# carlosmwh1985/BspAtom

Hardware: AMD Instinct MI355X
Metric: l-channel eigensolves/sec at N_bsp=4096 fp64 (higher is better)
Workload: dtype f64; 1 GPU; Hydrogen Coulomb l=0..127, N_bsp=4096, k=9, KIND_GRID=0 rb=800 (BASELINE configs[3]); `value` = weak scaling: 128 l-channels per GPU, 128 in total; channels_total=128, eigenvector_owner_rank=0, collective_calls=0, launched_by=python

## Files before the change

bspatom_amd/csrc/common.h:

```cpp
#pragma once
#include <hip/hip_runtime.h>
#include <cstdint>
#include <cstdio>
#include <cstdlib>

#define BSP_OK 0
#define BSP_ERR_HIP (-1)
#define BSP_ERR_ARG (-2)
#define BSP_ERR_BSPLVB (-3)
#define BSP_ERR_NOGPU (-4)
#define BSP_ERR_UNSUPPORTED (-5)

#define BSP_HIP(x)                                                                          \
    do {                                                                                    \
        hipError_t e_ = (x);                                                                \
        if (e_ != hipSuccess) {                                                             \
            fprintf(stderr, "bspatom: HIP error '%s' at %s:%d\n", hipGetErrorString(e_),    \
                    __FILE__, __LINE__);                                                    \
            return BSP_ERR_HIP;                                                             \
        }                                                                                   \
    } while (0)

typedef double double4_t __attribute__((ext_vector_type(4)));

__host__ __device__ inline size_t ab_stride(int npad) { return (size_t)npad * 128 + 1088; }

namespace bsp {

struct Options {
    int sb2st_version = 0;
    int sb2st_ring = 0;
    int sb2st_margin = 3, sb2st_hyst = 2;
    int sb2st_lead = 0;
    int sb2st_check = 0;
    int sb2st_diag = 0;
    int sb2st_force_abort = 0;
    int sy2sb_groups = 2, sy2sb_lookahead = 1, sy2sb_segs = 0;
    int panel_qr = 3;
    int tsqr_max_m = 2048;
    int tsqr_regcap = 1;
    int gemm_diag = 0;
    int bisect = 3, bisect_ept = 0;
    int bisect_secant = 1;
    int bisect_tail = 1;
    int no_eigvec_prefetch = 0;
    int vec_early = 1;
    int vec_own_cu = 1;
    int sb2sb_mfma = 1;
    int sb16_rows = 1;
    int poison_c = 0;
    int route = 0;
    int fused_probe = 0;
    int cw_items4 = 1;
    int cw_nw = 1;
    int cw_streams = 2;
    int cw_chunk_min = 1024;
    int s_overlap = 1;
    int cw_diag = 0;
    int cw_split = 0;
    int cw_band8 = 1;
    int sb8_wgs = 0;
    int cw_ipw = 0;
    int cw_ldspad = 0;
    int cw_onediv = 0;
    int ktime = 0;
};
Options &opts();

int process_device();
int process_device_check(int device);
void process_device_latch(int device);

enum KSlot { KS_SYR2K = 0, KS_SYMM, KS_PANEL_QR, KS_CHAIN, KS_SB2SB, KS_SB16ST, KS_BISECT, KS_STDFORM, KS_CRAWFORD, KS_COUNT };
void ktime_begin(int slot, hipStream_t st);
void ktime_end(int slot, hipStream_t st);
struct KScope {
    int slot; hipStream_t st; bool on;
    KScope(int slot_, hipStream_t st_) : slot(slot_), st(st_), on(opts().ktime != 0) { if (on) ktime_begin(slot, st); }
    ~KScope() { if (on) ktime_end(slot, st); }
};

struct GemmDesc {
    int M, N, K, batch;
    const double *A; long sAm, sAk, bA;
    const double *B; long sBk, sBn, bB;
    double *C; long sCm, sCn, bC;
    double alpha, beta;
    int lower_only;
    int yoff;
    int ksplit;
    int kchunk;
    long bCs;
    int nsb, toff;
    int sbpre[80];
    int sbxy[80];
};
int gemm_f64(const GemmDesc &g, hipStream_t st);
int gemm_splitk_f64(const GemmDesc &g, int splits, double *part, hipStream_t st);
int tsmm64_f64(int m, int batch, const double *A, long lda, long bsA, const double *B, long bsB, double *C, long ldc, long bsC,
               double alpha, double beta, hipStream_t st);
int syr2k_lower_f64(int m, int batch, double *A22, long ld, long bsA, const double *buf, long ldb, long bsBuf, int seg, int nseg,
                    int part, hipStream_t st);
int symm_lower_f64(int m, int batch, const double *A22, long ld, long bsA, const double *W, long ldw, long bsW,
                   double *Y, long ldy, long bsY, hipStream_t st);

int launch_point_table(int nkp, int k, int ka, int nfun, const double *d_rt, const double *d_aind,
                       const double *d_xg, const double *d_wg, const double *d_vpot, double *d_ptab,
                       int *d_left, int *d_status, hipStream_t st);
int launch_assemble_bands(int nfun, int k, int ka, int nkp, int kind_pot, const double *d_bl, int l0,
                          int nl, const double *d_ptab, const int *d_left, double *d_SB, double *d_HB,
                          hipStream_t st);
int launch_dipole_bands(int nfun, int k, int ka, int nkp, const double *d_ptab, const int *d_left, double *d_RB,
                        hipStream_t st);
int launch_band_cholesky(int n, int k, const double *d_SB, double *d_UB, double *d_rdiag, int *d_info,
                         hipStream_t st);
int launch_band_cholesky_range(int n, int k, int jstart, int jstop, const double *d_SB, double *d_UB, double *d_rdiag, int *d_info,
                               hipStream_t st);
int launch_band_cholesky_pair(int n, int k, int jstop, const double *d_SB, double *d_UB, double *d_rdiag, int *d_info, hipStream_t st);
int launch_standard_form(int n, int npad, int k, int nl, const double *d_HB, const double *d_UB,
                         const double *d_rdiag, double *d_Y, double *d_C, hipStream_t st, int full = 0);
struct CrawfordWork {
    double *SBf, *UBf, *rdiagf;
    double *Qel, *LiB;
    double *D, *E, *G;
    int *info;
};
bool crawford_supported(int n, int k);
size_t crawford_work_bytes(int n, int k, int nl);
void crawford_carve(void *base, int n, int k, int nl, CrawfordWork *w);
constexpr int CW_CHUNKS = 4;
int crawford_prepare(int n, int k, const double *d_SB, const CrawfordWork &w, hipStream_t st, hipEvent_t *evc = nullptr);
int crawford_run(int n, int npad, int k, int nl, const double *d_SB, const double *d_HB, const CrawfordWork &w, double *d_AB,
                 hipStream_t st, bool s_prepared = false, hipEvent_t *evc = nullptr, hipStream_t aux0 = nullptr);
long tsqr_scr_doubles(int npad);
long tsqr_cntr_ints(int npad);
int tsqr_panel(int npad, int r0, int c0, int batch, double *d_A, double *buf, double *W, double *scr, int *cntr, hipStream_t st);
struct Sy2sbWork {
    double *tsqr_scr;
    int *tsqr_cntr;
    double *buf2;
    double *tau2;
    double *buf;
    double *W;
    double *G;
    double *T;
    double *Kmat;
    double *tau;
    double *part;
};
constexpr int SY2SB_SPLITK = 16;
size_t sy2sb_work_bytes(int npad, int nb, int batch);
void sy2sb_carve(void *base, int npad, int nb, int batch, Sy2sbWork *w);
int sy2sb_run(int npad, int nb, int batch, double *d_A, const Sy2sbWork &w, hipStream_t st);
int sy2sb_panel_only(int npad, int c0, int batch, double *d_A, const Sy2sbWork &w, hipStream_t st);
int launch_extract_band(int npad, int nb, int batch, const double *d_A, double *d_AB, hipStream_t st);
size_t sb2st_ctl_bytes(int batch);
int launch_sb2sb(int n, int npad, int batch, double *d_AB, hipStream_t st);
int launch_sb16st(int n, int npad, int batch, double *d_AB, double *d_d, double *d_e, hipStream_t st, int *d_status = nullptr,
                  void *ctl = nullptr, int hb = 16);
int launch_sb2st(int n, int npad, int b, int batch, double *d_AB, double *d_d, double *d_e,
                 hipStream_t st, int *d_status = nullptr, void *ctl = nullptr);
int launch_bisect(int n, int ldn, int batch, const double *d_d, const double *d_e, double *d_w,
                  long ldw, hipStream_t st);
int launch_bisect_one(int n, const double *d_d, const double *d_e, int m, double *d_out, hipStream_t st);
int launch_band_multisect(int n, int k, const double *d_SB, const double *d_HB, int m, double *d_out, hipStream_t st);
constexpr size_t OWN_CU_LDS = 144 * 1024;
int launch_early_vector(int n, int k, const double *d_SB, const double *d_HB, int m, double *d_E, double *d_work, double *d_vec,
                        int *d_info, hipStream_t st, bool own_cu);
int launch_inverse_iteration(int n, int k, int nvec, const double *d_SB, const double *d_HB,
                             const int *d_chan, const double *d_E, double *d_work, double *d_vec,
                             int *d_info, hipStream_t st);
size_t invit_work_doubles(int n, int k);
size_t invit_batch_slot_doubles(int n, int k);
int invit_batch_slots(int k, int items, int *slots);
int launch_inverse_iteration_batch(int n, int k, int count, int items, int slots, const double *d_SB, const double *d_HB,
                                   const double *d_E, double *d_work, double *d_vec, int *d_info, hipStream_t st);
int launch_band_apply(int n, int k, const double *d_RB, const double a[3], const double *d_x, double *d_v, hipStream_t st);
int launch_dots(int n, int m, const double *d_Z, const double *d_v, double *d_D, hipStream_t st);
int launch_wf_tabulate(int nkp, int k, int n, const double *d_rt, const double *d_c, double ra,
                       double rb, int npts, double *d_r, double *d_u, int *d_status, hipStream_t st);

struct PipeBufs {
    double *UB, *rdiag, *Y, *C, *AB, *d, *e;
    void *work;
    int *info;
    int *status = nullptr;
    void *sbctl = nullptr;
    void *cwork = nullptr;
    hipEvent_t *s_events = nullptr;
    hipStream_t aux0 = nullptr;
    hipEvent_t chase_after = nullptr;
};
int pipeline_route(int n, int k);
size_t pipe_bytes_per_channel(int npad);
int pipeline_enqueue(int n, int npad, int k, int nl, const double *d_SB, const double *d_HB,
                     const PipeBufs &b, double *d_Eout, hipStream_t st, hipEvent_t *ev, bool with_bisect = true, bool s_prepared = false);

}
```

bspatom_amd/csrc/tridiag.hip:

```cpp
#include <vector>
#include "common.h"

namespace bsp {

__device__ __forceinline__ int sturm_count(const double *__restrict__ d, const double *__restrict__ e2,
                                           int n, double x, double pivmin)
{
    double q = d[0] - x;
    if (fabs(q) < pivmin) q = -pivmin;
    int cnt = (q < 0.0) ? 1 : 0;
    for (int i = 1; i < n; ++i) {
        q = (d[i] - x) - e2[i - 1] / q;
        if (fabs(q) < pivmin) q = -pivmin;
        cnt += (q < 0.0) ? 1 : 0;
    }
    return cnt;
}

constexpr int EPT = 4;

__global__ __launch_bounds__(256) void bisect_kernel(int n, int ldn, const double *__restrict__ dall,
                                                    const double *__restrict__ eall, double *wall, long ldw)
{
    extern __shared__ double sm[];
    double *d = sm, *e2 = sm + n;
    __shared__ double red[8];
    const int tid = threadIdx.x;
    const size_t ch = blockIdx.y;
    const double *dg = dall + ch * (size_t)ldn, *eg = eall + ch * (size_t)ldn;
    double gl = 1e300, gu = -1e300, emax = 0.0;
    for (int i = tid; i < n; i += 256) {
        const double di = dg[i];
        const double el = (i > 0) ? fabs(eg[i - 1]) : 0.0;
        const double er = (i < n - 1) ? fabs(eg[i]) : 0.0;
        d[i] = di;
        e2[i] = (i < n - 1) ? eg[i] * eg[i] : 0.0;
        gl = fmin(gl, di - el - er);
        gu = fmax(gu, di + el + er);
        emax = fmax(emax, er * er);
    }
#pragma unroll
    for (int off = 32; off >= 1; off >>= 1) {
        gl = fmin(gl, __shfl_xor(gl, off));
        gu = fmax(gu, __shfl_xor(gu, off));
        emax = fmax(emax, __shfl_xor(emax, off));
    }
    if ((tid & 63) == 0) { red[tid >> 6] = gl; red[4 + (tid >> 6)] = gu; }
    __syncthreads();
    gl = fmin(fmin(red[0], red[1]), fmin(red[2], red[3]));
    gu = fmax(fmax(red[4], red[5]), fmax(red[6], red[7]));
    __syncthreads();
    if ((tid & 63) == 0) red[tid >> 6] = emax;
    __syncthreads();
    emax = fmax(fmax(red[0], red[1]), fmax(red[2], red[3]));
    const double safmin = 2.2250738585072014e-308;
    const double pivmin = safmin * fmax(1.0, emax);
    const double tnorm = fmax(fabs(gl), fabs(gu));
    const double eps = 2.220446049250313e-16;
    gl = gl - 2.1 * tnorm * eps * n - 2.1 * pivmin;
    gu = gu + 2.1 * tnorm * eps * n + 2.1 * pivmin;

    const int mbase = blockIdx.x * (256 * EPT) + tid;
    double lo[EPT], hi[EPT];
#pragma unroll
    for (int c = 0; c < EPT; ++c) { lo[c] = gl; hi[c] = gu; }
    for (int it = 0; it < 128; ++it) {
        double mid[EPT];
        bool done[EPT];
        bool alld = true;
#pragma unroll
        for (int c = 0; c < EPT; ++c) {
            mid[c] = 0.5 * (lo[c] + hi[c]);
            done[c] = (mid[c] <= lo[c]) || (mid[c] >= hi[c]) ||
                      (hi[c] - lo[c] <= 2.0 * eps * fmax(fabs(lo[c]), fabs(hi[c])) + 2.0 * pivmin);
            alld = alld && done[c];
        }
        if (__syncthreads_and(alld)) break;
        double q[EPT];
        int cnt[EPT];
        {
            const double d0 = d[0];
#pragma unroll
            for (int c = 0; c < EPT; ++c) {
                q[c] = d0 - mid[c];
                if (fabs(q[c]) < pivmin) q[c] = -pivmin;
                cnt[c] = (q[c] < 0.0) ? 1 : 0;
            }
        }
        for (int i = 1; i < n; ++i) {
            const double di = d[i], ei = e2[i - 1];
#pragma unroll
            for (int c = 0; c < EPT; ++c) {
                double r = __builtin_amdgcn_rcp(q[c]);
                r = r * (2.0 - q[c] * r);
                q[c] = (di - mid[c]) - ei * r;
                if (fabs(q[c]) < pivmin) q[c] = -pivmin;
                cnt[c] += (q[c] < 0.0) ? 1 : 0;
            }
        }
#pragma unroll
        for (int c = 0; c < EPT; ++c) {
            if (!done[c]) {
                if (cnt[c] > mbase + 256 * c) hi[c] = mid[c]; else lo[c] = mid[c];
            }
        }
    }
#pragma unroll
    for (int c = 0; c < EPT; ++c) {
        const int m = mbase + 256 * c;
        if (m < n) wall[ch * (size_t)ldw + m] = 0.5 * (lo[c] + hi[c]);
    }
}

constexpr int RS = 8;

__global__ __launch_bounds__(256) void bisect2_kernel(int n, int ldn, const double *__restrict__ dall,
                                                     const double *__restrict__ eall, double *wall, long ldw)
{
    extern __shared__ double sm[];
    const int np = (n + RS - 1) / RS * RS;
    double *d = sm, *e2 = sm + np + RS;
    __shared__ double red[8];
    const int tid = threadIdx.x;
    const size_t ch = blockIdx.y;
    const double *dg = dall + ch * (size_t)ldn, *eg = eall + ch * (size_t)ldn;
    double gl = 1e300, gu = -1e300;
    for (int i = tid; i < n; i += 256) {
        const double di = dg[i];
        const double el = (i > 0) ? fabs(eg[i - 1]) : 0.0;
        const double er = (i < n - 1) ? fabs(eg[i]) : 0.0;
        gl = fmin(gl, di - el - er);
        gu = fmax(gu, di + el + er);
    }
#pragma unroll
    for (int off = 32; off >= 1; off >>= 1) {
        gl = fmin(gl, __shfl_xor(gl, off));
        gu = fmax(gu, __shfl_xor(gu, off));
    }
    if ((tid & 63) == 0) { red[tid >> 6] = gl; red[4 + (tid >> 6)] = gu; }
    __syncthreads();
    gl = fmin(fmin(red[0], red[1]), fmin(red[2], red[3]));
    gu = fmax(fmax(red[4], red[5]), fmax(red[6], red[7]));
    const double eps = 2.220446049250313e-16;
    double tnorm = fmax(fabs(gl), fabs(gu));
    if (!(tnorm > 0.0)) tnorm = 1.0;
    int kexp;
    (void)frexp(tnorm, &kexp);
    const double sc = ldexp(1.0, -kexp), isc = ldexp(1.0, kexp);
    for (int i = tid; i < np + RS; i += 256) {
        d[i] = (i < n) ? dg[i] * sc : 2.0;
        const double ev = (i < n - 1) ? (eg[i] * sc) : 0.0;
        e2[i] = fmax(ev * ev, 1e-60);
    }
    __syncthreads();
    gl = gl * sc - 2.1 * eps * n - 1e-300;
    gu = gu * sc + 2.1 * eps * n + 1e-300;

    const int mbase = blockIdx.x * (256 * EPT) + tid;
    double lo[EPT], hi[EPT];
#pragma unroll
    for (int c = 0; c < EPT; ++c) { lo[c] = gl; hi[c] = gu; }
    for (int it = 0; it < 128; ++it) {
        double mid[EPT];
        bool done[EPT];
        bool alld = true;
#pragma unroll
        for (int c = 0; c < EPT; ++c) {
            mid[c] = 0.5 * (lo[c] + hi[c]);
            done[c] = (mid[c] <= lo[c]) || (mid[c] >= hi[c]) ||
                      (hi[c] - lo[c] <= 2.0 * eps * fmax(fabs(lo[c]), fabs(hi[c])) + 1e-300);
            alld = alld && done[c];
        }
        if (__syncthreads_and(alld)) break;
        double p0[EPT], p1[EPT];
        int cnt[EPT];
#pragma unroll
        for (int c = 0; c < EPT; ++c) { p0[c] = 1.0; p1[c] = d[0] - mid[c]; cnt[c] = (p1[c] < 0.0) ? 1 : 0; }
        for (int ib = 0; ib < np; ib += RS) {
#pragma unroll
            for (int r = 0; r < RS; ++r) {
                const int i = ib + r + 1;
                const double di = d[i], ei = e2[i - 1];
#pragma unroll
                for (int c = 0; c < EPT; ++c) {
                    const double pn = __builtin_fma(di - mid[c], p1[c], -(ei * p0[c]));
                    cnt[c] += (int)((unsigned)(__double2hiint(pn) ^ __double2hiint(p1[c])) >> 31);
                    p0[c] = p1[c];
                    p1[c] = pn;
                }
            }
#pragma unroll
            for (int c = 0; c < EPT; ++c) {
                int ea, eb;
                (void)frexp(p1[c], &ea);
                (void)frexp(p0[c], &eb);
                const int ex = (p1[c] == 0.0) ? eb : ((p0[c] == 0.0) ? ea : max(ea, eb));
                p1[c] = ldexp(p1[c], -ex);
                p0[c] = ldexp(p0[c], -ex);
            }
        }
#pragma unroll
        for (int c = 0; c < EPT; ++c) {
            if (!done[c]) {
                if (cnt[c] > mbase + 256 * c) hi[c] = mid[c]; else lo[c] = mid[c];
            }
        }
    }
#pragma unroll
    for (int c = 0; c < EPT; ++c) {
        const int m = mbase + 256 * c;
        if (m < n) wall[ch * (size_t)ldw + m] = 0.5 * (lo[c] + hi[c]) * isc;
    }
}

constexpr int HW = 32;

#define STURM_BLOCK(LOADROW)                                                                          \
    {                                                                                                 \
        _Pragma("unroll") for (int sb = 0; sb < HW / RS; ++sb) {                                      \
            _Pragma("unroll") for (int r = 0; r < RS; ++r) {                                          \
                const double2 v = LOADROW(ib + sb * RS + r + 1);                                      \
                _Pragma("unroll") for (int c = 0; c < EPT; ++c) {                                     \
                    const double pn = __builtin_fma(v.x - x[c], p1[c], -(v.y * p0[c]));               \
                    h[c] = __builtin_amdgcn_alignbit(h[c], (unsigned)__double2hiint(pn), 31);         \
                    p0[c] = p1[c];                                                                    \
                    p1[c] = pn;                                                                       \
                }                                                                                     \
            }                                                                                         \
            _Pragma("unroll") for (int c = 0; c < EPT; ++c) {                                         \
                const int ex = -__builtin_amdgcn_frexp_exp(p1[c]);      \
                p1[c] = __builtin_amdgcn_ldexp(p1[c], ex);                                            \
                p0[c] = __builtin_amdgcn_ldexp(p0[c], ex);                                            \
                if (VAL) es[c] -= ex;                                            \
            }                                                                                         \
        }                                                                                             \
        _Pragma("unroll") for (int c = 0; c < EPT; ++c) {                                             \
            const unsigned t = __builtin_amdgcn_alignbit(hp[c], h[c], 1);                             \
            cnt[c] += __builtin_popcount(h[c] ^ t);                                                   \
            hp[c] = h[c];                                                                             \
        }                                                                                             \
    }
__device__ __forceinline__ double2 sturm_gload(const double2 *p)
{
    typedef double d2v __attribute__((ext_vector_type(2)));
    const d2v v = __builtin_nontemporal_load(reinterpret_cast<const d2v *>(p));
    return make_double2(v.x, v.y);
}
template <int EPT, bool VAL = false>
__device__ __forceinline__ void sturm_counts3(const double2 *__restrict__ de, int np, const double (&x)[EPT], int (&cnt)[EPT],
                                              const double2 *__restrict__ gt = nullptr, int nl = 0x7fffffff, float *lf = nullptr)
{
    double p0[EPT], p1[EPT];
    unsigned h[EPT], hp[EPT];
    int es[EPT];
#pragma unroll
    for (int c = 0; c < EPT; ++c) es[c] = 0;
    const double d0 = de[0].x;
#pragma unroll
    for (int c = 0; c < EPT; ++c) {
        p0[c] = 1.0; p1[c] = d0 - x[c];
        hp[c] = (unsigned)__double2hiint(p1[c]) >> 31;
        cnt[c] = (int)hp[c]; h[c] = 0u;
    }
    const int nlds = nl < np ? nl : np;
#define STURM_LDS(i) de[i]
#define STURM_GLB(i) sturm_gload(gt + (i))
    for (int ib = 0; ib < nlds; ib += HW) STURM_BLOCK(STURM_LDS)
    for (int ib = nlds; ib < np; ib += HW) STURM_BLOCK(STURM_GLB)
#undef STURM_LDS
#undef STURM_GLB
    if (VAL) {
#pragma unroll
        for (int c = 0; c < EPT; ++c) {
            const int e2 = __builtin_amdgcn_frexp_exp(p1[c]);
            const float mant = (float)__builtin_amdgcn_ldexp(p1[c], -e2);
            lf[c] = (float)(es[c] + e2) + __log2f(fmaxf(fabsf(mant), 1e-30f));
        }
    }
}

__device__ __forceinline__ double msect_point(double a, double w, int q, double rp)
{
    return __builtin_fma(w, (double)(q + 1) * rp, a);
}

__device__ __forceinline__ bool bracket_final(double lo, double hi)
{
    const double mid = 0.5 * (lo + hi);
    return (mid <= lo) || (mid >= hi) || (hi - lo <= 2.0 * 2.220446049250313e-16 * fmax(fabs(lo), fabs(hi)) + 1e-300);
}

static size_t bisect3_lds_bytes(int n, int ng)
{
    const int np = (n + HW - 1) / HW * HW;
    return (size_t)(np + 1) * 16 + (size_t)(ng / 2) * 16 + (size_t)ng * 4 + (size_t)(ng / 2) * 4;
}

template <int EPT, int TPB>
__global__ __launch_bounds__(TPB) void bisect3_kernel(int n, int ldn, const double *__restrict__ dall,
                                                     const double *__restrict__ eall, double *wall, long ldw, int tail,
                                                     double2 *gtail, int nl, int hybrid_arg)
{
    const int hybrid = EPT > 4 ? 0 : hybrid_arg;
    extern __shared__ double2 sde[];
    constexpr int NG = TPB * EPT;
    constexpr int NW = TPB / 64;
    constexpr int KC = NG / 2;
    const int np = (n + HW - 1) / HW * HW;
    const int nlr = nl < np ? nl : np;
    double2 *de = sde;
    const int kcap = hybrid ? NG / 4 : KC;
    double *llo = (double *)(sde + nlr + 1);
    double *lhi = llo + kcap;
    int *cg = (int *)(lhi + kcap);
    int *lm = cg + NG;
    __shared__ double red[2 * NW];
    __shared__ int sK;
    const int tid = threadIdx.x;
    const size_t ch = blockIdx.y;
    const double *dg = dall + ch * (size_t)ldn, *eg = eall + ch * (size_t)ldn;
    double *wout = wall + ch * (size_t)ldw;
    double2 *gt = gtail ? gtail + ch * (size_t)(np + 1) : nullptr;
    double gl = 1e300, gu = -1e300;
    for (int i = tid; i < n; i += TPB) {
        const double di = dg[i];
        const double el = (i > 0) ? fabs(eg[i - 1]) : 0.0;
        const double er = (i < n - 1) ? fabs(eg[i]) : 0.0;
        gl = fmin(gl, di - el - er);
        gu = fmax(gu, di + el + er);
    }
#pragma unroll
    for (int off = 32; off >= 1; off >>= 1) {
        gl = fmin(gl, __shfl_xor(gl, off));
        gu = fmax(gu, __shfl_xor(gu, off));
    }
    if ((tid & 63) == 0) { red[tid >> 6] = gl; red[NW + (tid >> 6)] = gu; }
    __syncthreads();
#pragma unroll
    for (int q = 0; q < NW; ++q) { gl = fmin(gl, red[q]); gu = fmax(gu, red[NW + q]); }
    const double eps = 2.220446049250313e-16;
    double tnorm = fmax(fabs(gl), fabs(gu));
    if (!(tnorm > 0.0)) tnorm = 1.0;
    int kexp;
    (void)frexp(tnorm, &kexp);
    const double sc = ldexp(1.0, -kexp), isc = ldexp(1.0, kexp);
    for (int i = tid; i <= np; i += TPB) {
        const double di = (i < n) ? dg[i] * sc : 2.0;
        const double ev = (i >= 1 && i < n) ? (eg[i - 1] * sc) : 0.0;
        const double2 row = make_double2(di, fmax(ev * ev, 1e-60));
        if (i <= nlr) de[i] = row; else gt[i] = row;
    }
    if (gt) asm volatile("s_waitcnt vmcnt(0)" ::: "memory");
    __syncthreads();
    gl = gl * sc - 2.1 * eps * n - 1e-300;
    gu = gu * sc + 2.1 * eps * n + 1e-300;

    const int mbase = blockIdx.x * NG + tid;
    double lo[EPT], hi[EPT];
    int clo[EPT], chi[EPT];
    float lflo[EPT], lfhi[EPT];
    if (!hybrid) {
        const double w = gu - gl;
        double xg[EPT];
        int cc[EPT];
#pragma unroll
        for (int c = 0; c < EPT; ++c) xg[c] = gl + w * ((double)(tid + TPB * c + 1) * (1.0 / (NG + 1)));
        sturm_counts3<EPT>(de, np, xg, cc, gt, nlr);
#pragma unroll
        for (int c = 0; c < EPT; ++c) cg[tid + TPB * c] = cc[c];
        __syncthreads();
#pragma unroll
        for (int c = 0; c < EPT; ++c) {
            const int m = mbase + TPB * c;
            int L = -1, R = NG;
            while (R - L > 1) {
                const int mid = (L + R) >> 1;
                if (cg[mid] > m) R = mid; else L = mid;
            }
            lo[c] = (L < 0) ? gl : gl + w * ((double)(L + 1) * (1.0 / (NG + 1)));
            hi[c] = (R >= NG) ? gu : gl + w * ((double)(R + 1) * (1.0 / (NG + 1)));
            clo[c] = (L < 0) ? 0 : cg[L];
            chi[c] = (R >= NG) ? n : cg[R];
        }
    }
    bool done[EPT];
    if (hybrid) {
        double *xs = llo;
        float *lfs = (float *)(xs + NG);
        unsigned short *cs = (unsigned short *)(lfs + NG);
        const int m0 = blockIdx.x * NG, m1 = min(m0 + NG, n);
        float wref[EPT];
        int st[EPT];
#pragma unroll
        for (int c = 0; c < EPT; ++c) {
            wref[c] = 3e38f; st[c] = 0;
            lo[c] = gl; hi[c] = gu; clo[c] = 0; chi[c] = n; lflo[c] = 3e38f; lfhi[c] = 3e38f;
        }
        for (int it = 0; it < 200; ++it) {
            double x[EPT];
            bool sec[EPT];
            int rng[EPT];
#pragma unroll
            for (int c = 0; c < EPT; ++c) {
                const int m = mbase + TPB * c;
                const double wd = hi[c] - lo[c];
                done[c] = (m >= n) || bracket_final(lo[c], hi[c]);
                if ((float)wd <= 0.5f * wref[c]) { wref[c] = (float)wd; st[c] &= 3; }
                const bool slow = (st[c] >> 2) >= 3;
                st[c] += 4;
                x[c] = 0.5 * (lo[c] + hi[c]); sec[c] = false; rng[c] = 0;
                const int a = max(clo[c], m0), b = min(chi[c], m1);
                if (chi[c] - clo[c] == 1 && lflo[c] < 1e38f && lfhi[c] < 1e38f && !slow && !done[c]) {
                    const double tiny = 2.0 * 2.220446049250313e-16 * fmax(fabs(lo[c]), fabs(hi[c]));
                    const float dl = fminf(fmaxf(lflo[c] - lfhi[c], -60.0f), 60.0f);
                    const double r = (double)exp2f(dl);
                    const double xe = fmin(fmax(lo[c] + wd * (r / (1.0 + r)), lo[c] + tiny), hi[c] - tiny);
                    if (xe > lo[c] && xe < hi[c]) { x[c] = xe; sec[c] = true; }
                } else if (b - a > 1 && m >= a && m < b && !slow && !done[c]) {
                    const double xq = msect_point(lo[c], wd, m - a, 1.0 / (double)(b - a + 1));
                    if (xq > lo[c] && xq < hi[c]) { x[c] = xq; rng[c] = (a - m0) | ((b - m0) << 16); }
                }
            }
            int tot = 0;
#pragma unroll
            for (int c = 0; c < EPT; ++c) tot += __syncthreads_count(!done[c]);
            if (tot <= (tail ? NG / hybrid : 0)) break;
            int cnt[EPT];
            float lf[EPT];
            sturm_counts3<EPT, true>(de, np, x, cnt, gt, nlr, lf);
#pragma unroll
            for (int c = 0; c < EPT; ++c) {
                xs[tid + TPB * c] = x[c]; cs[tid + TPB * c] = (unsigned short)cnt[c]; lfs[tid + TPB * c] = lf[c];
            }
            __syncthreads();
#pragma unroll
            for (int c = 0; c < EPT; ++c) {
                if (done[c]) continue;
                const int m = mbase + TPB * c;
                const bool up = cnt[c] > m;
                const int last = st[c] & 3;
                if (up) {
                    hi[c] = x[c]; chi[c] = cnt[c]; lfhi[c] = lf[c];
                    if (sec[c] && last == 1 && lflo[c] < 1e38f) lflo[c] -= 1.0f;
                } else {
                    lo[c] = x[c]; clo[c] = cnt[c]; lflo[c] = lf[c];
                    if (sec[c] && last == 2 && lfhi[c] < 1e38f) lfhi[c] -= 1.0f;
                }
                st[c] = (st[c] & ~3) | (sec[c] ? (up ? 1 : 2) : 0);
                if (rng[c]) {
                    const int s0 = rng[c] & 0xffff, s1 = rng[c] >> 16;
                    int L = s0 - 1, R = s1;
                    while (R - L > 1) {
                        const int mid = (L + R) >> 1;
                        if ((int)cs[mid] > m) R = mid; else L = mid;
                    }
                    if (R < s1) { const double xr = xs[R]; if (xr > lo[c] && xr < hi[c]) { hi[c] = xr; chi[c] = cs[R]; lfhi[c] = lfs[R]; } }
                    if (L >= s0) { const double xl = xs[L]; if (xl > lo[c] && xl < hi[c]) { lo[c] = xl; clo[c] = cs[L]; lflo[c] = lfs[L]; } }
                }
            }
        }
        __syncthreads();
    } else
    for (int it = 0; it < 160; ++it) {
        double mid[EPT];
        int nun = 0;
#pragma unroll
        for (int c = 0; c < EPT; ++c) {
            mid[c] = 0.5 * (lo[c] + hi[c]);
            done[c] = (mbase + TPB * c >= n) || bracket_final(lo[c], hi[c]);
            nun += done[c] ? 0 : 1;
        }
        if (!__syncthreads_or(nun > (tail ? EPT / 2 : 0))) break;
        int cnt[EPT];
        sturm_counts3<EPT>(de, np, mid, cnt, gt, nlr);
#pragma unroll
        for (int c = 0; c < EPT; ++c) {
            if (!done[c]) {
                if (cnt[c] > mbase + TPB * c) hi[c] = mid[c]; else lo[c] = mid[c];
            }
        }
    }
    if (tid == 0) sK = 0;
    __syncthreads();
#pragma unroll
    for (int c = 0; c < EPT; ++c) {
        const int m = mbase + TPB * c;
        done[c] = (m >= n) || bracket_final(lo[c], hi[c]);
        if (!done[c]) {
            const int pos = atomicAdd(&sK, 1);
            if (pos < kcap) { llo[pos] = lo[c]; lhi[pos] = hi[c]; lm[pos] = m; }
            else wout[m] = 0.5 * (lo[c] + hi[c]) * isc;
        } else if (m < n) wout[m] = 0.5 * (lo[c] + hi[c]) * isc;
    }
    __syncthreads();
    for (int round = 0; round < 128; ++round) {
        const int K = min(sK, kcap);
        if (K == 0) break;
        const int P = NG / K;
        const double rp = 1.0 / (double)(P + 1);
        double x[EPT];
        int cc[EPT];
#pragma unroll
        for (int c = 0; c < EPT; ++c) {
            const int s = tid + TPB * c, e = s / P, q = s - e * P;
            x[c] = 2.0;
            if (e < K) { const double a = llo[e]; x[c] = msect_point(a, lhi[e] - a, q, rp); }
        }
        sturm_counts3<EPT>(de, np, x, cc, gt, nlr);
#pragma unroll
        for (int c = 0; c < EPT; ++c) cg[tid + TPB * c] = cc[c];
        __syncthreads();
        double nlo[EPT / 2], nhi[EPT / 2];
        int nm[EPT / 2];
        bool keep[EPT / 2];
#pragma unroll
        for (int j = 0; j < EPT / 2; ++j) {
            const int e = tid + TPB * j;
            keep[j] = false;
            if (e < K) {
                const double a = llo[e], b = lhi[e], w = b - a;
                const int m = lm[e];
                const int *ce = cg + e * P;
                int L = -1, R = P;
                while (R - L > 1) {
                    const int mid = (L + R) >> 1;
                    if (ce[mid] > m) R = mid; else L = mid;
                }
                nlo[j] = (L < 0) ? a : msect_point(a, w, L, rp);
                nhi[j] = (R >= P) ? b : msect_point(a, w, R, rp);
                nm[j] = m;
                if (bracket_final(nlo[j], nhi[j]) || !(nhi[j] - nlo[j] < w)) wout[m] = 0.5 * (nlo[j] + nhi[j]) * isc;
                else keep[j] = true;
            }
        }
        __syncthreads();
        if (tid == 0) sK = 0;
        __syncthreads();
#pragma unroll
        for (int j = 0; j < EPT / 2; ++j) {
            if (keep[j]) {
                const int pos = atomicAdd(&sK, 1);
                llo[pos] = nlo[j]; lhi[pos] = nhi[j]; lm[pos] = nm[j];
            }
        }
        __syncthreads();
    }
    {
        const int K = min(sK, kcap);
        for (int e = tid; e < K; e += TPB) wout[lm[e]] = 0.5 * (llo[e] + lhi[e]) * isc;
    }
}

__global__ __launch_bounds__(64) void bisect_one_kernel(int n, const double *__restrict__ dg, const double *__restrict__ eg,
                                                       int m, double *out)
{
    extern __shared__ double sm[];
    const int np = (n + RS - 1) / RS * RS;
    double *d = sm, *e2 = sm + np + RS;
    const int lane = threadIdx.x;
    double gl = 1e300, gu = -1e300;
    for (int i = lane; i < n; i += 64) {
        const double di = dg[i];
        const double el = (i > 0) ? fabs(eg[i - 1]) : 0.0;
        const double er = (i < n - 1) ? fabs(eg[i]) : 0.0;
        gl = fmin(gl, di - el - er);
        gu = fmax(gu, di + el + er);
    }
#pragma unroll
    for (int off = 32; off >= 1; off >>= 1) {
        gl = fmin(gl, __shfl_xor(gl, off));
        gu = fmax(gu, __shfl_xor(gu, off));
    }
    const double eps = 2.220446049250313e-16;
    double tnorm = fmax(fabs(gl), fabs(gu));
    if (!(tnorm > 0.0)) tnorm = 1.0;
    int kexp;
    (void)frexp(tnorm, &kexp);
    const double sc = ldexp(1.0, -kexp), isc = ldexp(1.0, kexp);
    for (int i = lane; i < np + RS; i += 64) {
        d[i] = (i < n) ? dg[i] * sc : 2.0;
        const double ev = (i < n - 1) ? (eg[i] * sc) : 0.0;
        e2[i] = fmax(ev * ev, 1e-60);
    }
    __syncthreads();
    double lo = gl * sc - 2.1 * eps * n - 1e-300, hi = gu * sc + 2.1 * eps * n + 1e-300;
    for (int round = 0; round < 40; ++round) {
        if (hi - lo <= 2.0 * eps * fmax(fabs(lo), fabs(hi)) + 1e-300) break;
        const double w = (hi - lo) * (1.0 / 65.0);
        const double x = lo + (lane + 1) * w;
        if (!(x > lo && x < hi)) {
            const double mid = 0.5 * (lo + hi);
            if (!(mid > lo && mid < hi)) break;
        }
        double p0 = 1.0, p1 = d[0] - x;
        int cnt = (p1 < 0.0) ? 1 : 0;
        for (int ib = 0; ib < np; ib += RS) {
#pragma unroll
            for (int r = 0; r < RS; ++r) {
                const int i = ib + r + 1;
                const double pn = __builtin_fma(d[i] - x, p1, -(e2[i - 1] * p0));
                cnt += (int)((unsigned)(__double2hiint(pn) ^ __double2hiint(p1)) >> 31);
                p0 = p1; p1 = pn;
            }
            int ea, eb;
            (void)frexp(p1, &ea);
            (void)frexp(p0, &eb);
            const int ex = (p1 == 0.0) ? eb : ((p0 == 0.0) ? ea : max(ea, eb));
            p1 = ldexp(p1, -ex); p0 = ldexp(p0, -ex);
        }
        const unsigned long long above = __ballot(cnt > m);
        const int f = above ? (__ffsll((long long)above) - 1) : 64;
        const double xl = __shfl(x, f > 0 ? f - 1 : 0), xh = __shfl(x, f < 64 ? f : 63);
        const double nlo = (f > 0) ? xl : lo, nhi = (f < 64) ? xh : hi;
        if (!(nhi - nlo < hi - lo)) break;
        lo = nlo; hi = nhi;
    }
    if (lane == 0) *out = 0.5 * (lo + hi) * isc;
}

__global__ __launch_bounds__(256) void bisect_one3_kernel(int n, const double *__restrict__ dg, const double *__restrict__ eg,
                                                         int m, double *out)
{
    extern __shared__ double2 sde[];
    constexpr int NG = 256 * EPT;
    const int np = (n + HW - 1) / HW * HW;
    double2 *de = sde;
    int *cg = (int *)(sde + np + 1);
    __shared__ double red[8];
    const int tid = threadIdx.x;
    double gl = 1e300, gu = -1e300;
    for (int i = tid; i < n; i += 256) {
        const double di = dg[i];
        const double el = (i > 0) ? fabs(eg[i - 1]) : 0.0;
        const double er = (i < n - 1) ? fabs(eg[i]) : 0.0;
        gl = fmin(gl, di - el - er);
        gu = fmax(gu, di + el + er);
    }
#pragma unroll
    for (int off = 32; off >= 1; off >>= 1) {
        gl = fmin(gl, __shfl_xor(gl, off));
        gu = fmax(gu, __shfl_xor(gu, off));
    }
    if ((tid & 63) == 0) { red[tid >> 6] = gl; red[4 + (tid >> 6)] = gu; }
    __syncthreads();
    gl = fmin(fmin(red[0], red[1]), fmin(red[2], red[3]));
    gu = fmax(fmax(red[4], red[5]), fmax(red[6], red[7]));
    const double eps = 2.220446049250313e-16;
    double tnorm = fmax(fabs(gl), fabs(gu));
    if (!(tnorm > 0.0)) tnorm = 1.0;
    int kexp;
    (void)frexp(tnorm, &kexp);
    const double sc = ldexp(1.0, -kexp), isc = ldexp(1.0, kexp);
    for (int i = tid; i <= np; i += 256) {
        const double di = (i < n) ? dg[i] * sc : 2.0;
        const double ev = (i >= 1 && i < n) ? (eg[i - 1] * sc) : 0.0;
        de[i] = make_double2(di, fmax(ev * ev, 1e-60));
    }
    __syncthreads();
    double lo = gl * sc - 2.1 * eps * n - 1e-300, hi = gu * sc + 2.1 * eps * n + 1e-300;
    for (int round = 0; round < 24; ++round) {
        const double w = hi - lo;
        if (w <= 2.0 * eps * fmax(fabs(lo), fabs(hi)) + 1e-300) break;
        double x[EPT];
        int cc[EPT];
#pragma unroll
        for (int c = 0; c < EPT; ++c) x[c] = lo + w * ((double)(tid + 256 * c + 1) * (1.0 / (NG + 1)));
        sturm_counts3<EPT>(de, np, x, cc);
#pragma unroll
        for (int c = 0; c < EPT; ++c) cg[tid + 256 * c] = cc[c];
        __syncthreads();
        int L = -1, R = NG;
        while (R - L > 1) {
            const int mid = (L + R) >> 1;
            if (cg[mid] > m) R = mid; else L = mid;
        }
        __syncthreads();
        const double nlo = (L < 0) ? lo : lo + w * ((double)(L + 1) * (1.0 / (NG + 1)));
        const double nhi = (R >= NG) ? hi : lo + w * ((double)(R + 1) * (1.0 / (NG + 1)));
        if (!(nhi - nlo < w)) break;
        lo = nlo; hi = nhi;
    }
    if (tid == 0) *out = 0.5 * (lo + hi) * isc;
}

int launch_bisect_one(int n, const double *d_d, const double *d_e, int m, double *d_out, hipStream_t st)
{
    const int variant1 = opts().bisect;
    if (variant1 >= 3) {
        const size_t lds3 = (size_t)2 * (n + 3 * RS + HW) * sizeof(double) + 256 * EPT * sizeof(int);
        if (lds3 > 150 * 1024) return BSP_ERR_UNSUPPORTED;
        static bool attr3 = false;
        if (!attr3) {
            BSP_HIP(hipFuncSetAttribute(reinterpret_cast<const void *>(bisect_one3_kernel),
                                        hipFuncAttributeMaxDynamicSharedMemorySize, 150 * 1024));
            attr3 = true;
        }
        hipLaunchKernelGGL(bisect_one3_kernel, dim3(1), dim3(256), lds3, st, n, d_d, d_e, m, d_out);
        BSP_HIP(hipGetLastError());
        return BSP_OK;
    }
    const size_t lds = (size_t)2 * (n + 3 * RS) * sizeof(double);
    if (lds > 150 * 1024) return BSP_ERR_UNSUPPORTED;
    static bool attr = false;
    if (!attr) {
        BSP_HIP(hipFuncSetAttribute(reinterpret_cast<const void *>(bisect_one_kernel),
                                    hipFuncAttributeMaxDynamicSharedMemorySize, 150 * 1024));
        attr = true;
    }
    hipLaunchKernelGGL(bisect_one_kernel, dim3(1), dim3(64), lds, st, n, d_d, d_e, m, d_out);
    BSP_HIP(hipGetLastError());
    return BSP_OK;
}

int launch_bisect(int n, int ldn, int batch, const double *d_d, const double *d_e, double *d_w, long ldw,
                  hipStream_t st)
{
    const int ept_env = opts().bisect_ept;
    int mode = (ept_env == 8) ? 8 : (ept_env == 4) ? 4 : (ept_env == 2) ? 1024 : (ept_env == 21) ? 21 : (ept_env == 5) ? 512 : 22;
    int ng = (mode == 4) ? 1024 : (mode == 21 ? 512 : (mode == 22 ? 1024 : 2048));
    if (bisect3_lds_bytes(n, ng) > 150 * 1024) { mode = 22; ng = 1024; }
    const int np3 = (n + HW - 1) / HW * HW;
    int nl = np3;
    while (bisect3_lds_bytes(nl, ng) > 150 * 1024) nl -= HW;
    const size_t lds3 = bisect3_lds_bytes(nl, ng);
    const size_t lds = (size_t)2 * (n + 3 * RS + HW) * sizeof(double);
    struct Tail { hipStream_t st; double2 *p; size_t cap; };
    static std::vector<Tail> g_tails;
    double2 *gtail = nullptr;
    if (nl < np3) {
        const size_t need = (size_t)batch * (np3 + 1);
        Tail *tl = nullptr;
        for (auto &x : g_tails) if (x.st == st) tl = &x;
        if (!tl) { g_tails.push_back({st, nullptr, 0}); tl = &g_tails.back(); }
        if (need > tl->cap) {
            if (tl->p) { BSP_HIP(hipStreamSynchronize(st)); (void)hipFree(tl->p); tl->p = nullptr; tl->cap = 0; }
            BSP_HIP(hipMalloc(reinterpret_cast<void **>(&tl->p), need * sizeof(double2)));
            tl->cap = need;
        }
        gtail = tl->p;
        if (opts().bisect < 3) return BSP_ERR_UNSUPPORTED;
    }
    static bool attr_set = false;
    const int variant = opts().bisect;
    if (!attr_set) {
        BSP_HIP(hipFuncSetAttribute(reinterpret_cast<const void *>(bisect_kernel),
                                    hipFuncAttributeMaxDynamicSharedMemorySize, 150 * 1024));
        BSP_HIP(hipFuncSetAttribute(reinterpret_cast<const void *>(bisect2_kernel),
                                    hipFuncAttributeMaxDynamicSharedMemorySize, 150 * 1024));
        BSP_HIP(hipFuncSetAttribute(reinterpret_cast<const void *>(bisect3_kernel<4, 256>),
                                    hipFuncAttributeMaxDynamicSharedMemorySize, 150 * 1024));
        BSP_HIP(hipFuncSetAttribute(reinterpret_cast<const void *>(bisect3_kernel<8, 256>),
                                    hipFuncAttributeMaxDynamicSharedMemorySize, 150 * 1024));
        BSP_HIP(hipFuncSetAttribute(reinterpret_cast<const void *>(bisect3_kernel<4, 512>),
                                    hipFuncAttributeMaxDynamicSharedMemorySize, 150 * 1024));
        BSP_HIP(hipFuncSetAttribute(reinterpret_cast<const void *>(bisect3_kernel<2, 1024>),
                                    hipFuncAttributeMaxDynamicSharedMemorySize, 150 * 1024));
        BSP_HIP(hipFuncSetAttribute(reinterpret_cast<const void *>(bisect3_kernel<2, 256>),
                                    hipFuncAttributeMaxDynamicSharedMemorySize, 150 * 1024));
        BSP_HIP(hipFuncSetAttribute(reinterpret_cast<const void *>(bisect3_kernel<2, 512>),
                                    hipFuncAttributeMaxDynamicSharedMemorySize, 150 * 1024));
        attr_set = true;
    }
    const dim3 grid((n + 256 * EPT - 1) / (256 * EPT), batch);
    KScope kt(KS_BISECT, st);
    if (variant == 1) hipLaunchKernelGGL(bisect_kernel, grid, dim3(256), lds, st, n, ldn, d_d, d_e, d_w, ldw);
    else if (variant == 2) hipLaunchKernelGGL(bisect2_kernel, grid, dim3(256), lds, st, n, ldn, d_d, d_e, d_w, ldw);
    else {
        const dim3 g3((n + ng - 1) / ng, batch);
        const int tail = opts().bisect_tail;
        const int hyb = n > 65535 ? 0 : (opts().bisect_secant == 1 ? 8 : (opts().bisect_secant >= 4 ? opts().bisect_secant : (opts().bisect_secant >= 2 ? 4 : 0)));
        if (mode == 512) hipLaunchKernelGGL((bisect3_kernel<4, 512>), g3, dim3(512), lds3, st, n, ldn, d_d, d_e, d_w, ldw, tail, gtail, nl, hyb);
        else if (mode == 1024) hipLaunchKernelGGL((bisect3_kernel<2, 1024>), g3, dim3(1024), lds3, st, n, ldn, d_d, d_e, d_w, ldw, tail, gtail, nl, hyb);
        else if (mode == 8) hipLaunchKernelGGL((bisect3_kernel<8, 256>), g3, dim3(256), lds3, st, n, ldn, d_d, d_e, d_w, ldw, tail, gtail, nl, hyb);
        else if (mode == 21) hipLaunchKernelGGL((bisect3_kernel<2, 256>), g3, dim3(256), lds3, st, n, ldn, d_d, d_e, d_w, ldw, tail, gtail, nl, hyb);
        else if (mode == 22) hipLaunchKernelGGL((bisect3_kernel<2, 512>), g3, dim3(512), lds3, st, n, ldn, d_d, d_e, d_w, ldw, tail, gtail, nl, hyb);
        else hipLaunchKernelGGL((bisect3_kernel<4, 256>), g3, dim3(256), lds3, st, n, ldn, d_d, d_e, d_w, ldw, tail, gtail, nl, hyb);
    }
    BSP_HIP(hipGetLastError());
    return BSP_OK;
}

}
```

Baseline: 1879 eigensolves/s.

## Add compacted tail Sturm evaluation and budgeted multisection to hybrid bisection

Restructures the hybrid bisection loop so unconverged eigenvalue lanes can be compacted into a dense list via wave ballots. Sturm counts are then evaluated only for active points, and results are exchanged through LDS. It also adds a reduced-thread budget mode for the final multisection rounds. The intent is to avoid spending full-block Sturm sweeps on mostly finished eigenvalues. The default tail mode is changed to 2, which keeps the compaction and budget paths off. The default path gains extra LDS traffic and barriers.

```diff
diff --git a/bspatom_amd/csrc/common.h b/bspatom_amd/csrc/common.h
--- a/bspatom_amd/csrc/common.h
+++ b/bspatom_amd/csrc/common.h
@@ -42,7 +42,7 @@
     int gemm_diag = 0;
     int bisect = 3, bisect_ept = 0;
     int bisect_secant = 1;
-    int bisect_tail = 1;
+    int bisect_tail = 2;
     int no_eigvec_prefetch = 0;
     int vec_early = 1;
     int vec_own_cu = 1;
diff --git a/bspatom_amd/csrc/tridiag.hip b/bspatom_amd/csrc/tridiag.hip
--- a/bspatom_amd/csrc/tridiag.hip
+++ b/bspatom_amd/csrc/tridiag.hip
@@ -293,7 +293,7 @@
 static size_t bisect3_lds_bytes(int n, int ng)
 {
     const int np = (n + HW - 1) / HW * HW;
-    return (size_t)(np + 1) * 16 + (size_t)(ng / 2) * 16 + (size_t)ng * 4 + (size_t)(ng / 2) * 4;
+    return (size_t)(np + 1) * 16 + (size_t)(ng / 2) * 16 + (size_t)ng * 4 + (size_t)(ng / 2) * 4 + (size_t)(ng - ng / 4) * 2;
 }
 
 template <int EPT, int TPB>
@@ -314,8 +314,11 @@
     double *lhi = llo + kcap;
     int *cg = (int *)(lhi + kcap);
     int *lm = cg + NG;
-    __shared__ double red[2 * NW];
+    __shared__ double red[(EPT > 4 ? EPT / 2 : 2) * NW];
     __shared__ int sK;
+    constexpr int KT = 16;
+    constexpr int BUD = 128;
+    constexpr bool NEWTAIL = EPT <= 2;
     const int tid = threadIdx.x;
     const size_t ch = blockIdx.y;
     const double *dg = dall + ch * (size_t)ldn, *eg = eall + ch * (size_t)ldn;
@@ -388,6 +391,12 @@
         double *xs = llo;
         float *lfs = (float *)(xs + NG);
         unsigned short *cs = (unsigned short *)(lfs + NG);
+        unsigned short *lst = cs + NG;
+        constexpr int LC = NG - NG / 4;
+        int *wcnt = (int *)red;
+        const int lane = tid & 63, wv = tid >> 6;
+        const bool compacting = NEWTAIL && (tail == 1 || tail == 3);
+        const int handover = (NEWTAIL && tail == 1) ? KT : ((tail == 1 || tail == 2) ? NG / hybrid : 0);
         const int m0 = blockIdx.x * NG, m1 = min(m0 + NG, n);
         float wref[EPT];
         int st[EPT];
@@ -421,18 +430,67 @@
                     if (xq > lo[c] && xq < hi[c]) { x[c] = xq; rng[c] = (a - m0) | ((b - m0) << 16); }
                 }
             }
-            int tot = 0;
-#pragma unroll
-            for (int c = 0; c < EPT; ++c) tot += __syncthreads_count(!done[c]);
-            if (tot <= (tail ? NG / hybrid : 0)) break;
+            unsigned long long bal[EPT];
+#pragma unroll
+            for (int c = 0; c < EPT; ++c) {
+                bal[c] = __ballot(!done[c]);
+                if (lane == 0) wcnt[c * NW + wv] = __popcll(bal[c]);
+            }
+            __syncthreads();
+            int tot = 0, pre[EPT];
+#pragma unroll
+            for (int c = 0; c < EPT; ++c) {
+#pragma unroll
+                for (int q = 0; q < NW; ++q) {
+                    if (q == wv) pre[c] = tot;
+                    tot += wcnt[c * NW + q];
+                }
+            }
+            if (tot <= handover) break;
+            const bool compact = compacting && tot <= LC;
+            const double qnan = __longlong_as_double(0x7ff8000000000000ll);
+#pragma unroll
+            for (int c = 0; c < EPT; ++c) {
+                xs[tid + TPB * c] = (compact && done[c]) ? qnan : x[c];
+                if (compact && !done[c])
+                    lst[pre[c] + __popcll(bal[c] & ((1ull << lane) - 1ull))] = (unsigned short)(tid + TPB * c);
+            }
+            __syncthreads();
+            if (!NEWTAIL) {
+                int ce[EPT];
+                float le[EPT];
+                sturm_counts3<EPT, true>(de, np, x, ce, gt, nlr, le);
+#pragma unroll
+                for (int c = 0; c < EPT; ++c) { cs[tid + TPB * c] = (unsigned short)ce[c]; lfs[tid + TPB * c] = le[c]; }
+            } else if (compact && tot <= TPB) {
+                if (wv * 64 < tot) {
+                    const int s = (tid < tot) ? (int)lst[tid] : -1;
+                    const double x1[1] = {s >= 0 ? xs[s] : 2.0};
+                    int c1[1];
+                    float l1[1];
+                    sturm_counts3<1, true>(de, np, x1, c1, gt, nlr, l1);
+                    if (s >= 0) { cs[s] = (unsigned short)c1[0]; lfs[s] = l1[0]; }
+                }
+            } else if (!compact || wv * 64 * EPT < tot) {
+                int se[EPT], ce[EPT];
+                double xe[EPT];
+                float le[EPT];
+#pragma unroll
+                for (int c = 0; c < EPT; ++c) {
+                    const int e = (wv * EPT + c) * 64 + lane;
+                    se[c] = compact ? (e < tot ? (int)lst[e] : -1) : tid + TPB * c;
+                    xe[c] = compact ? (se[c] >= 0 ? xs[se[c]] : 2.0) : x[c];
+                }
+                sturm_counts3<EPT, true>(de, np, xe, ce, gt, nlr, le);
+#pragma unroll
+                for (int c = 0; c < EPT; ++c)
+                    if (se[c] >= 0) { cs[se[c]] = (unsigned short)ce[c]; lfs[se[c]] = le[c]; }
+            }
+            __syncthreads();
             int cnt[EPT];
             float lf[EPT];
-            sturm_counts3<EPT, true>(de, np, x, cnt, gt, nlr, lf);
-#pragma unroll
-            for (int c = 0; c < EPT; ++c) {
-                xs[tid + TPB * c] = x[c]; cs[tid + TPB * c] = (unsigned short)cnt[c]; lfs[tid + TPB * c] = lf[c];
-            }
-            __syncthreads();
+#pragma unroll
+            for (int c = 0; c < EPT; ++c) { cnt[c] = cs[tid + TPB * c]; lf[c] = lfs[tid + TPB * c]; }
 #pragma unroll
             for (int c = 0; c < EPT; ++c) {
                 if (done[c]) continue;
@@ -470,7 +528,7 @@
             done[c] = (mbase + TPB * c >= n) || bracket_final(lo[c], hi[c]);
             nun += done[c] ? 0 : 1;
         }
-        if (!__syncthreads_or(nun > (tail ? EPT / 2 : 0))) break;
+        if (!__syncthreads_or(nun > ((tail == 1 || tail == 2) ? EPT / 2 : 0))) break;
         int cnt[EPT];
         sturm_counts3<EPT>(de, np, mid, cnt, gt, nlr);
 #pragma unroll
@@ -496,19 +554,31 @@
     for (int round = 0; round < 128; ++round) {
         const int K = min(sK, kcap);
         if (K == 0) break;
-        const int P = NG / K;
+        const bool budget = NEWTAIL && hybrid && tail == 1 && K <= BUD;
+        const int P = (budget ? BUD : NG) / K;
         const double rp = 1.0 / (double)(P + 1);
-        double x[EPT];
-        int cc[EPT];
-#pragma unroll
-        for (int c = 0; c < EPT; ++c) {
-            const int s = tid + TPB * c, e = s / P, q = s - e * P;
-            x[c] = 2.0;
-            if (e < K) { const double a = llo[e]; x[c] = msect_point(a, lhi[e] - a, q, rp); }
-        }
-        sturm_counts3<EPT>(de, np, x, cc, gt, nlr);
-#pragma unroll
-        for (int c = 0; c < EPT; ++c) cg[tid + TPB * c] = cc[c];
+        if (budget) {
+            if (tid < BUD) {
+                const int e = tid / P, q = tid - e * P;
+                double x1[1] = {2.0};
+                int c1[1];
+                if (e < K) { const double a = llo[e]; x1[0] = msect_point(a, lhi[e] - a, q, rp); }
+                sturm_counts3<1>(de, np, x1, c1, gt, nlr);
+                cg[tid] = c1[0];
+            }
+        } else {
+            double x[EPT];
+            int cc[EPT];
+#pragma unroll
+            for (int c = 0; c < EPT; ++c) {
+                const int s = tid + TPB * c, e = s / P, q = s - e * P;
+                x[c] = 2.0;
+                if (e < K) { const double a = llo[e]; x[c] = msect_point(a, lhi[e] - a, q, rp); }
+            }
+            sturm_counts3<EPT>(de, np, x, cc, gt, nlr);
+#pragma unroll
+            for (int c = 0; c < EPT; ++c) cg[tid + TPB * c] = cc[c];
+        }
         __syncthreads();
         double nlo[EPT / 2], nhi[EPT / 2];
         int nm[EPT / 2];
```

After: 1879 eigensolves/s (median of 3 runs). About the same (-0.0%).
